# leonsick/depthg

Measured on AMD Instinct MI355X. Metric: correlation-loss steps/sec at B=32,C=384,28x28 (fwd+bwd, per-GPU batch 32), higher is better.
Workload: dtype bf16 (feats) / f16 (code) MFMA inputs, f32 accumulate

## Files before the change

depthg_amd/csrc/dg_corr_args.h:

```cpp
#pragma once
#include "dg_device.h"

__host__ __device__ inline int dg_perm32(int pl) {
    int s = pl >> 4, u = (pl >> 3) & 1, hh = (pl >> 2) & 1, v = pl & 3;
    return (2 * s + hh) * 8 + 4 * u + v;
}

#ifndef DG_F_IG
#define DG_F_IG 4
#endif
__host__ __device__ inline int dg_f_off(int q, int g) {
    constexpr int IG = DG_F_IG;
    return ((g / IG) * 32 + q) * (IG * 16) + (((g % IG) ^ ((q / (16 / IG)) % IG)) * 16);
}

struct DgBlob {
    int GF, GD, KD;
    int off_c, off_p, bytes;
    __host__ __device__ DgBlob(int KF, int KD_) : GF(KF / 8), GD(KD_ / 8), KD(KD_) {
        off_c = 32 * GF * 16;
        off_p = off_c + GD * 32 * 16;
        bytes = off_p + 4 * KD * 16;
    }
    __host__ __device__ int f(int q, int g) const { return dg_f_off(q, g); }
    __host__ __device__ int c(int q, int g) const { return off_c + (g * 32 + q) * 16; }
    __host__ __device__ int p(int d, int cc) const { return off_p + (cc * KD + d) * 16; }
};

template <int NKF, int NKD>
struct BlobT {
    static constexpr int KF = NKF * 16, KD = NKD * 16, GF = KF / 8, GD = KD / 8;
    static constexpr int OFF_C = 32 * GF * 16;
    static constexpr int OFF_P = OFF_C + GD * 32 * 16;
    static constexpr int BYTES = OFF_P + 4 * KD * 16;
    static constexpr int CHUNKS = BYTES / 1024;
    static constexpr int CHUNK_C0 = OFF_C / 1024;
    static constexpr int CHUNK_P0 = OFF_P / 1024;
    static_assert(BYTES % 1024 == 0 && OFF_C % 1024 == 0 && OFF_P % 1024 == 0, "blob parts must be KiB multiples");
    static_assert(GF % 16 == 0, "swizzle needs 16-granule groups");
};

__host__ __device__ inline size_t dg_gtile_off(int p, int d, int DP) {
    const int q = p & 31;
    return ((size_t)(p >> 5) * (DP >> 5) + (d >> 5)) * 1024 + (q >> 3) * 256 + ((d & 31) + 32 * ((q >> 2) & 1)) * 4 + (q & 3);
}

#define DG_XROWS_LDS (4 * 33 * 16)
template <int NDF>
__device__ __forceinline__ void dg_load_code_rows(const char* Cp, char* T, int lane, _Float16 (&x)[NDF][16]) {
        const int r = lane & 31, h = lane >> 5;
    i32x4 raw[NDF][2];
#pragma unroll
    for (int f = 0; f < NDF; ++f)
#pragma unroll
        for (int k = 0; k < 2; ++k) raw[f][k] = *reinterpret_cast<const i32x4*>(Cp + f * 2048 + k * 1024 + lane * 16);
#pragma unroll
    for (int f = 0; f < NDF; ++f) {
#pragma unroll
        for (int k = 0; k < 2; ++k) {
            const int L = k * 64 + lane;
            *reinterpret_cast<i32x4*>(T + ((L >> 5) * 33 + (L & 31)) * 16) = raw[f][k];
        }
#pragma unroll
        for (int i = 0; i < 16; ++i) {
            const int q = (i & 3) + 8 * (i >> 2) + 4 * h;
            x[f][i] = *reinterpret_cast<const _Float16*>(T + ((r >> 3) * 33 + q) * 16 + (r & 7) * 2);
        }
    }
}

enum { DG_JOB_HELPER = 0, DG_JOB_DEPTH = 1 };

struct DgJob {
    const char* Rop;
    const char* Sop;
    const float* rvec;
    const float* rimg;
    const uint32_t* maskbits;
    const float* nzR;
    const float* nzS;
    const float* RcInv;
    const float* Scsum;
    const int64_t* ridx;
    const int64_t* sidx;
    float* dR;
    float* part;
    float* out_cd;
    float* out_loss;
    uint16_t* Gout;
    float shift;
    int32_t kind;
    int32_t center_on_lane;
    int32_t slot_loss;
    int32_t slot_cd;
    float fin_scale;
    int32_t fold;
};

#define DG_MAX_JOBS 12
#define DG_GR_CAP 24

struct DgCorrArgs {
    DgJob jobs[DG_MAX_JOBS];
    int32_t njobs;
    int32_t B, P, Ppad;
    int32_t nrb;
    int32_t D;
    float lo, hi;
    float inv_BP;
    const char* dummy;
    int32_t pos_w;
    uint32_t* wctr;
    unsigned long long* span;
    int32_t half_tiles;
    uint32_t* stamps;
    unsigned long long* blocklog;
    const int32_t* gr_list;
    const int32_t* gr_count;
    const int16_t* gr_rank;
    int32_t gr_nkeys, gr_cpb;
    int32_t gr_blocks_per_image;
    int8_t gr_key[DG_MAX_JOBS];
    int8_t gr_first[DG_MAX_JOBS];
    int32_t gr_nblk[DG_MAX_JOBS];
};

struct DgFinishArgs {
    const float* part[DG_MAX_JOBS];
    int32_t slot_loss[DG_MAX_JOBS];
    int32_t slot_cd[DG_MAX_JOBS];
    float scale[DG_MAX_JOBS];
    int32_t njobs, nblk, B, P;
    int32_t nblk_job[DG_MAX_JOBS];
    const float* nzsum;
    float* out;
    float wtot[4];
};


struct DgTransposeArgs {
    const float* src[5];
    float* dst[5];
    int32_t K[5], K4[5], HW[5];
    int32_t nmaps;
};

struct DgGatherJob {
    const float* src;
    const float* coords;
    const int64_t* srcidx;
    char* blob;
    float* inv_norm;
    float* colpart;
    int32_t K, K4, Kpad;
    int32_t is_code;
    int32_t h, w;
    const float* ext_inv;
};
#define DG_MAX_GATHER 20
struct DgPreArgs {
    uint64_t seed; unsigned long long* state; int64_t* perms; int32_t count;
    const float* depth; float* nz; float* nzsum; int32_t dH, dW;
    const float* coords1; const float* coords2; char* taps;
    int32_t B, h, w, S, Sh, P, Ppad;
    unsigned int* zero_word;
};

struct DgCdMaskArgs {
    const float* rowsR;
    const float* rowsS[DG_MAX_NEG + 2];
    const int64_t* sidx[DG_MAX_NEG + 2];
    uint32_t* bits[DG_MAX_NEG + 2];
    int32_t T, B, P, Ppad, D, D4;
};

struct DgGatherArgs {
    DgGatherJob jobs[DG_MAX_GATHER];
    int32_t njobs, B, S, Sh, P, Ppad, KF, KD;
    int32_t direct;
    DgCdMaskArgs cd;
    int32_t cd_xper;
    DgPreArgs pre;
    int32_t pre_blocks, pre_nz, pre_z0;
};

struct DgPlaneArgs {
    const float* src[4];
    int32_t K[4], K4[4];
    float* rows[DG_MAX_NEG + 2][2];
    const float* coords1;
    const float* coords2;
    const int64_t* perms;
    int32_t nops, B, h, w, S, Sh, P;
    int32_t tap_consumers;
    int32_t feats_bf16;
    const float* src_x;
    float* rows_x;
};

__device__ __forceinline__ void dg_super_perm_row(const float* __restrict__ keys, uint64_t seed, unsigned long long* __restrict__ state,
                                                  int B, int64_t* __restrict__ out, int row, int nrows, float* sk) {
    const float* kr = keys ? keys + (size_t)row * B : nullptr;
    unsigned long long draw = 0;
    if (state) { seed = state[0]; draw = state[1]; }
    const uint64_t key = seed + 0x9E3779B97F4A7C15ull * draw;
    for (int i = threadIdx.x; i < B; i += 256)
        sk[i] = kr ? kr[i] : (float)(dg_philox(key, (uint32_t)(row * B + i)) >> 8) * (1.0f / 16777216.0f);
    __syncthreads();
    for (int i = threadIdx.x; i < B; i += 256) {
        const float ki = sk[i];
        int rank = 0;
        for (int j = 0; j < B; ++j) rank += (sk[j] < ki) || (sk[j] == ki && j < i);
        out[(size_t)row * B + rank] = (int64_t)((i == rank ? i + 1 : i) % B);
    }
    if (state && threadIdx.x == 0) {
        __threadfence();
        if (atomicAdd(&state[2], 1ull) == (unsigned long long)nrows - 1) {
            state[1] = draw + 1;
            state[2] = 0;
            __threadfence();
        }
    }
}

__device__ __forceinline__ float depth_nz_at(const float* __restrict__ depth, int n, int p, int H, int W, int Sh, int S) {
    float out = 0.f;
    if (p < Sh * S) {
        const int i = p / S, j = p - i * S;
        const float sy = Sh > 1 ? (float)(H - 1) / (float)(Sh - 1) : 0.f;
        const float sx = S > 1 ? (float)(W - 1) / (float)(S - 1) : 0.f;
        const float fy = dg_mul_rn(sy, (float)i), fx = dg_mul_rn(sx, (float)j);
        int y0 = min((int)fy, H - 1), x0 = min((int)fx, W - 1);
        const int y1 = y0 < H - 1 ? y0 + 1 : y0, x1 = x0 < W - 1 ? x0 + 1 : x0;
        const float ly1 = fy - (float)y0, lx1 = fx - (float)x0, ly0 = 1.f - ly1, lx0 = 1.f - lx1;
        const float* d = depth + (size_t)n * H * W;
        const float top = dg_mul_rn(d[(size_t)y0 * W + x0], lx0) + dg_mul_rn(d[(size_t)y0 * W + x1], lx1);
        const float bot = dg_mul_rn(d[(size_t)y1 * W + x0], lx0) + dg_mul_rn(d[(size_t)y1 * W + x1], lx1);
        const float v = dg_mul_rn(top, ly0) + dg_mul_rn(bot, ly1);
        out = v / fmaxf(fabsf(v), DG_EPS_NORM);
    }
    return out;
}

__device__ __forceinline__ void depth_nz_image(const float* __restrict__ depth, float* __restrict__ nz, float* __restrict__ nzsum,
                                               int n, int H, int W, int Sh, int S, int Ppad, bool pixel_order = false) {
    __shared__ float wred[4];
    float s = 0.f;
    for (int p = threadIdx.x; p < Ppad; p += 256) {
        const int pref = (pixel_order && p < Sh * S) ? (p % S) * S + p / S : p;
        const float v = depth_nz_at(depth, n, pref, H, W, Sh, S);
        nz[(size_t)n * Ppad + p] = v;
        s += v;
    }
#pragma unroll
    for (int o = 32; o > 0; o >>= 1) s += __shfl_xor(s, o, 64);
    if ((threadIdx.x & 63) == 0) wred[threadIdx.x >> 6] = s;
    __syncthreads();
    if (threadIdx.x == 0) nzsum[n] = wred[0] + wred[1] + wred[2] + wred[3];
}

struct DgSmallArgs {
    const void* rowsF[DG_MAX_NEG + 2];
    const float* rowsC[DG_MAX_NEG + 2];
    int32_t T, B, P, Ppad, C4, D, D4, KD;
    int32_t opR[DG_MAX_NEG + 2];
    int32_t opS[DG_MAX_NEG + 2];
    const int64_t* sidx[DG_MAX_NEG + 2];
    int32_t pointwise, depth, grad;
    float lo, hi;
    float shift[DG_MAX_NEG + 2], shift_depth;
    const float* nz;
    const float* nzsum;
    float* dRA[DG_MAX_NEG + 3];
    float* dRA2[DG_MAX_NEG + 2];
    float* dRB[DG_MAX_NEG + 2][2];
    float* dRB2[DG_MAX_NEG + 2][2];
    float* part;
    float* om;
    unsigned int* ticket;
    char* xop;
    float* xinv;
    int32_t blob_bytes, blob_off_c;
    float* out;
    float wtot[4];
    int32_t nsplit;
    float* out_cd;
    float* out_loss;
    int32_t mat_t, mat;
    int32_t debug;
    unsigned long long* span;
};

struct DgGatherRowsArgs {
    const float* src[2 * (DG_MAX_NEG + 2)];
    const float* coords[2 * (DG_MAX_NEG + 2)];
    const int64_t* srcidx[2 * (DG_MAX_NEG + 2)];
    void* rows[2 * (DG_MAX_NEG + 2)];
    int32_t K4[2 * (DG_MAX_NEG + 2)], h[2 * (DG_MAX_NEG + 2)], w[2 * (DG_MAX_NEG + 2)];
    int32_t Kout[2 * (DG_MAX_NEG + 2)], as_bf16[2 * (DG_MAX_NEG + 2)];
    int32_t njobs, B, S, Sh, P;
};

struct DgDenseArgs {
    const float* src[2];
    const float* code[2];
    char* blob[2];
    float* colpart[2];
    float* inv_norm[2];
    float* ccolpart[2];
    const float* depth;
    float* nz;
    float* nzsum;
    int32_t B, K, D, KF, KD, h, w, P, Ppad, dH, dW;
    int64_t* draw_out;
    unsigned long long* draw_state;
    uint64_t draw_seed;
    int32_t draw_count;
    int32_t code_split;
    const float* fkeep[2];
    float fscale;
    int32_t unit;
    int32_t roles;
};

struct DgDenseCodeArgs {
    const float* code[2];
    char* blob[2];
    const float* inv_norm[2];
    float* ccolpart[2];
    int32_t B, D, KF, KD, h, w, P, Ppad;
    char* clo[2];
};

struct DgGroupArgs {
    const int64_t* sidx[DG_MAX_JOBS];
    int8_t key[DG_MAX_JOBS];
    int32_t nh, nkeys, B;
    int32_t* list;
    int32_t* count;
    int16_t* rank;
};
__device__ __forceinline__ void dg_group_lists(const DgGroupArgs& g, const int m, const int key, const int lane) {
    const int B = g.B;
    int src[DG_MAX_JOBS];
#pragma unroll
    for (int j = 0; j < DG_MAX_JOBS; ++j) {
        const bool mine = j < g.nh && g.key[j] == key && lane < B;
        const int64_t* sidx = mine ? g.sidx[j] : nullptr;
        src[j] = mine ? (sidx ? (int)sidx[lane] : lane) : -1;
    }
    int cnt = 0;
#pragma unroll
    for (int j = 0; j < DG_MAX_JOBS; ++j) {
        const bool hit = src[j] == m;
        const unsigned long long mask = __ballot(hit);
        if (hit) {
            const int rk = cnt + __popcll(mask & ((1ull << lane) - 1ull));
            g.rank[j * B + lane] = (int16_t)(rk < 32767 ? rk : 32767);
            if (rk < DG_GR_CAP) g.list[(key * B + m) * DG_GR_CAP + rk] = j | (lane << 8);
        }
        cnt += __popcll(mask);
    }
    if (lane == 0) g.count[key * B + m] = cnt < DG_GR_CAP ? cnt : DG_GR_CAP;
}

struct DgColmeanArgs {
    const float* colpart[DG_MAX_NEG + 2];
    float* bbar[DG_MAX_NEG + 2];
    __bf16* bsplit[DG_MAX_NEG + 2];
    const float* ccolpart[DG_MAX_NEG + 2];
    float* csum[DG_MAX_NEG + 2];
// ... 154 lines not shown
```

depthg_amd/csrc/dg_post.hip:

```cpp
#include "dg_device.h"
#include "dg_corr_args.h"
#include "dg_taps.h"
#include <cstdlib>

typedef const float __attribute__((address_space(1)))* gfloat_p;


#define DG_LOAD_GS(a, gs)                                                                                   \
    float gs[4];                                                                                            \
    {                                                                                                       \
        const bool vec_ = (a).gscal != nullptr;                                                             \
        const float gt_ = vec_ ? (a).gscal[DG_OUT_TOTAL] : (a).gtot[0];                                     \
        const float g0_ = vec_ ? (a).gscal[0] : 0.f, g1_ = vec_ ? (a).gscal[1] : 0.f;                       \
        const float g2_ = vec_ ? (a).gscal[2] : 0.f, g3_ = vec_ ? (a).gscal[3] : 0.f;                       \
        gs[0] = g0_ + gt_ * (a).wtot[0]; gs[1] = g1_ + gt_ * (a).wtot[1];                                  \
        gs[2] = g2_ + gt_ * (a).wtot[2]; gs[3] = g3_ + gt_ * (a).wtot[3];                                  \
    }
__device__ __forceinline__ float dg_pick(const float (&gs)[4], int i) { return i == 0 ? gs[0] : (i == 1 ? gs[1] : (i == 2 ? gs[2] : gs[3])); }

template <int NDF>
__global__ __launch_bounds__(64 * NDF) void k_grad_combine(const DgScatterArgs a) {
    const int rt = blockIdx.x, n = blockIdx.y, dest = blockIdx.z;
    const int lane = threadIdx.x & 63, r = lane & 31, h = lane >> 5, DP = NDF * 32;
    const int d = __builtin_amdgcn_readfirstlane((int)threadIdx.x >> 6);
    if (dest >= 2) {
        const int j = dest - 2;
        const size_t off = ((size_t)n * (a.Ppad >> 5) + rt) * (32 * DP) + d * 1024 + lane * 4;
        const float f = a.axf[j] ? a.axf[j][0] : 0.f;
        const float* const d2 = a.axd2[j];
        const float* const s1 = a.axs[j];
        const float* const s2 = a.axs2[j];
        f32x4 y[4], y2[4], x[4], x2[4];
#pragma unroll
        for (int g = 0; g < 4; ++g) {
            y[g] = *reinterpret_cast<const f32x4*>(a.axd[j] + off + g * 256);
            y2[g] = d2 ? *reinterpret_cast<const f32x4*>(d2 + off + g * 256) : f32x4{0.f, 0.f, 0.f, 0.f};
            x[g] = s1 ? *reinterpret_cast<const f32x4*>(s1 + off + g * 256) : f32x4{0.f, 0.f, 0.f, 0.f};
            x2[g] = s2 ? *reinterpret_cast<const f32x4*>(s2 + off + g * 256) : f32x4{0.f, 0.f, 0.f, 0.f};
        }
#pragma unroll
        for (int g = 0; g < 4; ++g) {
#pragma unroll
            for (int e = 0; e < 4; ++e) y[g][e] = fmaf(f, x[g][e] + x2[g][e], y[g][e] + y2[g][e]);
            *reinterpret_cast<f32x4*>(a.axo[j] + off + g * 256) = y[g];
        }
        return;
    }
    __shared__ __attribute__((aligned(16))) char xs[NDF][DG_XROWS_LDS];
    __shared__ float part[NDF][32];
    DG_LOAD_GS(a, gs)
    const bool ok = 32 * d + r < a.D;
    const size_t tile_off = ((size_t)n * (a.Ppad >> 5) + rt) * (32 * DP) + lane * 4 + (ok ? d * 1024 : 0);
    float v[16];
#pragma unroll
    for (int i = 0; i < 16; ++i) v[i] = 0.f;
    auto add_sources = [&](const int8_t* list, const int cnt) __attribute__((always_inline)) {
        for (int k0 = 0; k0 < cnt; k0 += 4) {
            f32x4 t[4][4];
            float sc[4];
#pragma unroll
            for (int u = 0; u < 4; ++u) {
                const bool live = k0 + u < cnt;
                const DgScatterSrc& q = a.src[(int)list[live ? k0 + u : k0]];
                sc[u] = live ? dg_src_factor(q) * dg_pick(gs, q.gidx) : 0.f;
                const float* base = q.buf + tile_off;
#pragma unroll
                for (int g = 0; g < 4; ++g) t[u][g] = *reinterpret_cast<const f32x4*>(base + (ok ? g * 256 : 0));
            }
#pragma unroll
            for (int u = 0; u < 4; ++u) {
                const bool use = ok && k0 + u < cnt;
#pragma unroll
                for (int g = 0; g < 4; ++g)
#pragma unroll
                    for (int e = 0; e < 4; ++e) v[4 * g + e] = fmaf(sc[u], use ? t[u][g][e] : 0.f, v[4 * g + e]);
            }
        }
    };
    const int nraw = a.ncraw[dest];
    add_sources(a.craw[dest], nraw);
    if (nraw > 0) {
        const char* xb = a.xop + ((size_t)n * (a.Ppad >> 5) + rt) * a.blob_bytes + a.blob_off_c + d * 2048;
        _Float16 x[1][16];
        dg_load_code_rows<1>(xb, xs[d], lane, x);
#pragma unroll
        for (int i = 0; i < 16; ++i) {
            const float t = half_sum((float)x[0][i] * v[i]);
            if (r == 0) part[d][h * 16 + i] = t;
        }
        __syncthreads();
#pragma unroll
        for (int i = 0; i < 16; ++i) {
            float t = part[0][h * 16 + i];
#pragma unroll
            for (int f = 1; f < NDF; ++f) t += part[f][h * 16 + i];
            const int rr = rt * 32 + (i & 3) + 8 * (i >> 2) + 4 * h;
            const float inv = rr < a.P ? a.xinv[(size_t)n * a.Ppad + rr] : 0.f;
            v[i] = (v[i] - (float)x[0][i] * t) * inv;
        }
    }
    add_sources(a.cfin[dest], a.ncfin[dest]);
    if (ok) {
        float* out = a.comb[dest] + tile_off;
#pragma unroll
        for (int g = 0; g < 4; ++g) {
            const f32x4 t = {v[4 * g], v[4 * g + 1], v[4 * g + 2], v[4 * g + 3]};
            *reinterpret_cast<f32x4*>(out + g * 256) = t;
        }
    }
}

#ifndef COMB_HB_HM
#define COMB_HB_HM 4
#endif
#ifndef COMB_HB
#define COMB_HB 4
#endif
#define COMB_MAXROUTE 512
template <int NDF, bool HM = false>
__global__ __launch_bounds__(64 * NDF) void k_combine_out(const DgScatterArgs a) {
    const int rt = blockIdx.x, n = blockIdx.y, dest = blockIdx.z;
    const int tid = threadIdx.x, lane = tid & 63, r = lane & 31, h = lane >> 5, DP = NDF * 32;
    const int d = __builtin_amdgcn_readfirstlane(tid >> 6);
    __shared__ __attribute__((aligned(16))) char xs[NDF][DG_XROWS_LDS];
    __shared__ float part[NDF][32];
    __shared__ float stage[NDF][32 * 33];
    __shared__ const float* rl_p[COMB_MAXROUTE];
    __shared__ float rl_w[COMB_MAXROUTE];
    __shared__ int rl_cnt, wcnt[NDF], rsrc[DG_MAX_SCATTER];
    DG_LOAD_GS(a, gs)
    int nr = 0;
    for (int s = 0; s < a.nsrc; ++s)
        if (a.src[s].dest == dest && a.src[s].route != nullptr) { if (tid == 0) rsrc[nr] = s; ++nr; }
    if (tid == 0) rl_cnt = 0;
    __syncthreads();
    for (int i0 = 0; i0 < nr * a.B; i0 += 64 * NDF) {
        const int i = i0 + tid;
        bool hit = false;
        int m = 0, s = 0;
        if (i < nr * a.B) {
            const int rs = i / a.B;
            m = i - rs * a.B; s = rsrc[rs];
            hit = (int)a.src[s].route[m] == n;
        }
        const unsigned long long bal = __ballot(hit);
        if (lane == 0) wcnt[d] = __popcll(bal);
        __syncthreads();
        int base = rl_cnt;
        for (int wv = 0; wv < d; ++wv) base += wcnt[wv];
        if (hit) {
            const int o = base + __popcll(bal & ((1ull << lane) - 1));
            const DgScatterSrc& q = a.src[s];
            if (o < COMB_MAXROUTE) {
                rl_p[o] = q.half ? reinterpret_cast<const float*>(reinterpret_cast<const _Float16*>(q.buf) + (size_t)m * a.Ppad * a.DP) : q.buf + (size_t)m * a.Ppad * a.DP;
                rl_w[o] = dg_src_factor(q) * dg_pick(gs, q.gidx);
            }
        }
        __syncthreads();
        if (tid == 0) {
            int c = rl_cnt;
            for (int wv = 0; wv < NDF; ++wv) c += wcnt[wv];
            rl_cnt = min(c, COMB_MAXROUTE);
        }
        __syncthreads();
    }
    const int cnt = rl_cnt;
    const bool ok = 32 * d + r < a.D;
    const size_t in_img = (size_t)rt * (32 * DP) + lane * 4 + (ok ? d * 1024 : 0);
    const size_t tile_off = (size_t)n * a.Ppad * DP + in_img;
    float v[16];
#pragma unroll
    for (int i = 0; i < 16; ++i) v[i] = 0.f;
    const size_t in_img_h = (size_t)rt * (32 * DP) + lane * 8 + (ok ? d * 1024 : 0);
    constexpr int HB = HM ? COMB_HB_HM : COMB_HB, FB = HM ? 1 : 4;
    float invd[16];
#pragma unroll
    for (int i = 0; i < 16; ++i) {
        const int rr = rt * 32 + (i & 3) + 8 * (i >> 2) + 4 * h;
        invd[i] = (a.xinv_dest[dest] && rr < a.P) ? a.xinv_dest[dest][(size_t)n * a.Ppad + rr] : 0.f;
    }
    const _Float16 __attribute__((address_space(1)))* const hdummy = reinterpret_cast<const _Float16 __attribute__((address_space(1)))*>(reinterpret_cast<uintptr_t>(a.xinv));
    auto add_half4 = [&](const _Float16 __attribute__((address_space(1)))* const (&hb)[HB], const float (&sc)[HB], const bool raw) __attribute__((always_inline)) {
        f16x8 t0[HB], t1[HB];
#pragma unroll
        for (int u = 0; u < HB; ++u) {
            t0[u] = *reinterpret_cast<const f16x8 __attribute__((address_space(1)))*>(hb[u]);
            t1[u] = *reinterpret_cast<const f16x8 __attribute__((address_space(1)))*>(hb[u] + ((ok && hb[u] != hdummy) ? 512 : 0));
        }
#pragma unroll
        for (int u = 0; u < HB; ++u) {
            const bool use = ok && sc[u] != 0.f;
#pragma unroll
            for (int e = 0; e < 8; ++e) {
                v[e] = fmaf(raw ? sc[u] : sc[u] * invd[e], use ? (float)t0[u][e] : 0.f, v[e]);
                v[8 + e] = fmaf(raw ? sc[u] : sc[u] * invd[8 + e], use ? (float)t1[u][e] : 0.f, v[8 + e]);
            }
        }
    };
    auto add_sources_half = [&](const int8_t* list, const int nsrc_, const bool raw) __attribute__((always_inline)) {
        for (int k0 = 0; k0 < nsrc_; k0 += HB) {
            const _Float16 __attribute__((address_space(1)))* hb[HB];
            float sc[HB];
#pragma unroll
            for (int u = 0; u < HB; ++u) {
                const bool live = k0 + u < nsrc_;
                const DgScatterSrc& q = a.src[(int)list[live ? k0 + u : k0]];
                sc[u] = live ? dg_src_factor(q) * dg_pick(gs, q.gidx) : 0.f;
                hb[u] = live ? reinterpret_cast<const _Float16 __attribute__((address_space(1)))*>(reinterpret_cast<uintptr_t>(q.buf)) + (size_t)n * a.Ppad * DP + in_img_h
                             : hdummy;
            }
            add_half4(hb, sc, raw);
        }
    };
    auto add_sources = [&](const int8_t* list, const int nsrc_) __attribute__((always_inline)) {

        for (int k0 = 0; k0 < nsrc_; k0 += FB) {
            f32x4 t[FB][4];
            float sc[FB];
#pragma unroll
            for (int u = 0; u < FB; ++u) {
                const bool live = k0 + u < nsrc_;
                const DgScatterSrc& q = a.src[(int)list[live ? k0 + u : k0]];
                sc[u] = live ? dg_src_factor(q) * dg_pick(gs, q.gidx) : 0.f;
                const float* base = q.buf + tile_off;
#pragma unroll
                for (int g = 0; g < 4; ++g) t[u][g] = *reinterpret_cast<const f32x4*>(base + (ok ? g * 256 : 0));
            }
#pragma unroll
            for (int u = 0; u < FB; ++u) {
                const bool use = ok && k0 + u < nsrc_;
#pragma unroll
                for (int g = 0; g < 4; ++g)
#pragma unroll
                    for (int e = 0; e < 4; ++e) v[4 * g + e] = fmaf(sc[u], use ? t[u][g][e] : 0.f, v[4 * g + e]);
            }
        }
    };
    const int nraw = a.ncraw[dest] + a.ncrawh[dest];
    add_sources(a.craw[dest], a.ncraw[dest]);
    add_sources_half(a.crawh[dest], a.ncrawh[dest], true);
    if (nraw > 0) {
        const char* xb = a.xop + ((size_t)n * (a.Ppad >> 5) + rt) * a.blob_bytes + a.blob_off_c + d * 2048;
        _Float16 x[1][16];
        dg_load_code_rows<1>(xb, xs[d], lane, x);
#pragma unroll
        for (int i = 0; i < 16; ++i) {
            const float t = half_sum((float)x[0][i] * v[i]);
            if (r == 0) part[d][h * 16 + i] = t;
        }
        __syncthreads();
#pragma unroll
        for (int i = 0; i < 16; ++i) {
            float t = part[0][h * 16 + i];
#pragma unroll
            for (int f = 1; f < NDF; ++f) t += part[f][h * 16 + i];
            const int rr = rt * 32 + (i & 3) + 8 * (i >> 2) + 4 * h;
            const float inv = rr < a.P ? a.xinv[(size_t)n * a.Ppad + rr] : 0.f;
            v[i] = (v[i] - (float)x[0][i] * t) * inv;
        }
    }
    add_sources(a.cfin[dest], a.ncfin[dest]);
    add_sources_half(a.cfinh[dest], a.ncfinh[dest], false);
    if (a.routed_half) {
        for (int e0 = 0; e0 < cnt; e0 += HB) {
            const _Float16 __attribute__((address_space(1)))* hb[HB];
            float sc[HB];
#pragma unroll
            for (int k = 0; k < HB; ++k) {
                const int e = min(e0 + k, cnt - 1);
                sc[k] = e0 + k < cnt ? rl_w[e] : 0.f;
                hb[k] = sc[k] != 0.f ? reinterpret_cast<const _Float16 __attribute__((address_space(1)))*>(reinterpret_cast<uintptr_t>(rl_p[e])) + in_img_h : hdummy;
            }
            add_half4(hb, sc, false);
        }
    } else
    for (int e0 = 0; e0 < cnt; e0 += 4) {
        f32x4 u4[4][4];
        float sc[4];
#pragma unroll
        for (int k = 0; k < 4; ++k) {
            const int e = min(e0 + k, cnt - 1);
            sc[k] = e0 + k < cnt ? rl_w[e] : 0.f;
            const gfloat_p sb = (gfloat_p)rl_p[e] + in_img;
#pragma unroll
            for (int g = 0; g < 4; ++g) u4[k][g] = *(const f32x4 __attribute__((address_space(1)))*)(sb + (ok ? g * 256 : 0));
        }
#pragma unroll
        for (int k = 0; k < 4; ++k)
#pragma unroll
            for (int g = 0; g < 4; ++g)
#pragma unroll
                for (int e = 0; e < 4; ++e) v[4 * g + e] = fmaf(sc[k], ok ? u4[k][g][e] : 0.f, v[4 * g + e]);
    }
    float* st = stage[d];
#pragma unroll
    for (int i = 0; i < 16; ++i) st[r * 33 + (i & 3) + 8 * (i >> 2) + 4 * h] = v[i];
    __builtin_amdgcn_fence(__ATOMIC_RELEASE, "workgroup");
    __builtin_amdgcn_wave_barrier();
    __builtin_amdgcn_fence(__ATOMIC_ACQUIRE, "workgroup");
    const int HW = a.h * a.w, p = rt * 32 + r;
    float* out = a.out[dest] + (size_t)n * a.D * HW + p;
#pragma unroll
    for (int it = 0; it < 16; ++it) {
        const int c = 2 * it + h, ch = 32 * d + c;
        if (ch < a.D && p < a.P) out[(size_t)ch * HW] = st[c * 33 + r];
    }
}

#define SCAT_THREADS 1024
#define SCAT_DC 4
#define SCAT_PX (SCAT_THREADS / SCAT_DC)
#define SCAT_MAXPASS 16

__global__ __launch_bounds__(SCAT_THREADS) void k_build_taps(const DgScatterArgs a) {
    extern __shared__ __attribute__((aligned(16))) char sg[];
    const DgTapsArgs t{a.coords1, a.coords2, a.taps, a.B, a.h, a.w, a.S, a.Sh, a.P};
    build_taps_block<SCAT_THREADS>(t, (int)blockIdx.x, (int)blockIdx.y, sg);
}

__global__ __launch_bounds__(256) void k_pre_general(const DgPreArgs a) {
    extern __shared__ __attribute__((aligned(16))) char pg[];
    int b = (int)blockIdx.x;
    if (a.zero_word && b == 0 && threadIdx.x == 0) *a.zero_word = 0u;
    if (b < a.count) { dg_super_perm_row(nullptr, a.seed, a.state, a.B, a.perms, b, a.count, reinterpret_cast<float*>(pg)); return; }
    b -= a.count;
    if (a.depth) {
        if (b < a.B) { depth_nz_image(a.depth, a.nz, a.nzsum, b, a.dH, a.dW, a.Sh, a.S, a.Ppad); return; }
        b -= a.B;
    }
    if (!a.taps) return;
    const DgTapsArgs t{a.coords1, a.coords2, a.taps, a.B, a.h, a.w, a.S, a.Sh, a.P};
    build_taps_block<256>(t, b % a.B, b / a.B, pg);
}

hipError_t dg_launch_pre_general(const DgPreArgs& a, hipStream_t s) {
    int nblk = a.count + (a.depth ? a.B : 0) + (a.taps ? 2 * a.B : 0);
    if (nblk == 0 && a.zero_word) nblk = 1;
    if (nblk == 0) return hipSuccess;
    size_t smem = a.count > 0 ? (size_t)a.B * 4 : 0;
    if (a.taps) {
        const size_t need = dg_taps_record_bytes(a.h * a.w, a.P) + (size_t)a.h * a.w * 4 + 16;
        smem = need > smem ? need : smem;
    }
    return dg_launch(k_pre_general, dim3(nblk), dim3(256), (int)smem, s, a);
}

#define SCAT_RMAX 8
template <int NPASS>
__global__ __launch_bounds__(SCAT_THREADS) void k_scatter_grad(const DgScatterArgs a, int rmax) {
    extern __shared__ __attribute__((aligned(16))) char sg[];
    const int tid = threadIdx.x, HW = a.h * a.w, P = a.P;
    const int aD = a.D, aDP = a.DP, aB = a.B, aPpad = a.Ppad;
    const char* const taps_base = a.taps;
    DG_LOAD_GS(a, gs)
    const int dc0 = blockIdx.x * SCAT_DC, bdst = blockIdx.y, dest = blockIdx.z;
    const int dl = tid & (SCAT_DC - 1), px = tid / SCAT_DC, d = dc0 + dl;
    const int npass = (HW + SCAT_PX - 1) / SCAT_PX;
    const size_t rec = dg_taps_record_bytes(HW, P);
    __shared__ const float* b_src[SCAT_RMAX];
    __shared__ const char* b_rec[SCAT_RMAX];
    __shared__ float b_sc[SCAT_RMAX];
    float acc[NPASS];
#pragma unroll
    for (int i = 0; i < NPASS; ++i) acc[i] = 0.f;
    int npend = 0;

    auto flush = [&, aD, aDP]() __attribute__((always_inline)) {
        if (npend == 0) return;
        __syncthreads();
        const int n16 = (int)(rec / 16);
        for (int i = tid; i < npend * n16; i += SCAT_THREADS) {
            const int r = i / n16, k = i - r * n16;
            reinterpret_cast<f32x4*>(sg)[i] = *((const f32x4 __attribute__((address_space(1)))*)b_rec[r] + k);
        }
        __syncthreads();
        if (d < aD) {
            const int DPc = aDP;
            constexpr int RG = NPASS <= 4 ? 4 : (NPASS <= 8 ? 2 : 1);
            for (int r0 = 0; r0 < npend; r0 += RG) {
                float v[RG][NPASS], w[RG][NPASS];
                int e0[RG][NPASS];
#pragma unroll
                for (int g = 0; g < RG; ++g) {
                    const int r = min(r0 + g, npend - 1);
                    const int* off = reinterpret_cast<const int*>(sg + (size_t)r * rec);
                    const float* ewgt = reinterpret_cast<const float*>(off + HW + 1);
                    const unsigned short* eidx = reinterpret_cast<const unsigned short*>(ewgt + 4 * P);
                    const gfloat_p src = (gfloat_p)b_src[r];
#pragma unroll
                    for (int ps = 0; ps < NPASS; ++ps) {
                        const int pix = ps * SCAT_PX + px;
                        const bool ok = r0 + g < npend && ps < npass && pix < HW;
                        const int ea = ok ? off[pix] : 0, eb = ok ? off[pix + 1] : 0;
                        const bool any = eb > ea;
                        w[g][ps] = any ? ewgt[ea] : 0.f;
                        v[g][ps] = any ? src[dg_gtile_off(eidx[ea], d, DPc)] : 0.f;
                        e0[g][ps] = ea | (eb > ea + 1 ? (int)0x80000000 : 0);
                    }
                }
#pragma unroll
                for (int g = 0; g < RG; ++g) {
                    if (r0 + g < npend) {
                        const int r = r0 + g;
                        const int* off = reinterpret_cast<const int*>(sg + (size_t)r * rec);
                        const float* ewgt = reinterpret_cast<const float*>(off + HW + 1);
                        const unsigned short* eidx = reinterpret_cast<const unsigned short*>(ewgt + 4 * P);
                        const gfloat_p src = (gfloat_p)b_src[r];
                        const float sc = b_sc[r];
#pragma unroll
                        for (int ps = 0; ps < NPASS; ++ps) {
                            float sum = w[g][ps] * v[g][ps];
                            if (e0[g][ps] < 0) {
                                const int ea = e0[g][ps] & 0x7fffffff, eb = off[ps * SCAT_PX + px + 1];
                                for (int e = ea + 1; e < eb; ++e) sum = fmaf(ewgt[e], src[dg_gtile_off(eidx[e], d, DPc)], sum);
                            }
                            acc[ps] = fmaf(sc, sum, acc[ps]);
                        }
                    }
                }
            }
        }
        __syncthreads();
        npend = 0;
    };
    auto push = [&](const float* buf, float sc, int cs, int nimg) __attribute__((always_inline)) {
        if (tid == 0) {
            b_src[npend] = buf + (size_t)nimg * aPpad * aDP;
            b_rec[npend] = taps_base + ((size_t)cs * aB + nimg) * rec;
            b_sc[npend] = sc;
        }
        if (++npend == rmax) flush();
    };

    push(a.comb[dest], 1.0f, dest == 0 ? 0 : 1, bdst);
    for (int s = 0; s < a.nsrc; ++s) {
        const DgScatterSrc& q = a.src[s];
        if (q.dest != dest || q.route == nullptr) continue;
        const float sc = dg_src_factor(q) * dg_pick(gs, q.gidx);
        for (int n0 = 0; n0 < a.B; n0 += 64) {
            const int nn = n0 + (tid & 63);
            const bool hit = nn < a.B && (int)q.route[nn] == bdst;
            unsigned long long m = __ballot(hit);
            while (m) {
                const int n = n0 + __builtin_ctzll(m);
                m &= m - 1;
                push(q.buf, sc, q.coords_sel, n);
            }
        }
    }
    flush();
    float* stage = reinterpret_cast<float*>(sg);
#pragma unroll
    for (int ps = 0; ps < NPASS; ++ps) {
        const int pix = ps * SCAT_PX + px;
        if (ps < npass && pix < HW) stage[dl * (HW + 1) + pix] = acc[ps];
    }
    __syncthreads();
    float* out = a.out[dest];
    for (int i = tid; i < SCAT_DC * HW; i += SCAT_THREADS) {
        const int dd = i / HW, pix = i - dd * HW;
        if (dc0 + dd < a.D) out[((size_t)bdst * a.D + dc0 + dd) * HW + pix] = stage[dd * (HW + 1) + pix];
    }
}

template <int CG>
__global__ __launch_bounds__(SCAT_THREADS) void k_scatter_small(const DgScatterArgs a, int rb) {
    constexpr int VS = CG + 1;
    extern __shared__ __attribute__((aligned(16))) char sg[];
    const int tid = threadIdx.x, HW = a.h * a.w, P = a.P, nt = a.Ppad >> 5, NF = a.DP >> 5;
    const int aB = a.B, aPpad = a.Ppad, aDP = a.DP;
    const char* const taps_base = a.taps;
    DG_LOAD_GS(a, gs)
    const int f = blockIdx.x / (32 / CG), cg = blockIdx.x % (32 / CG), bdst = blockIdx.y, dest = blockIdx.z;
    const size_t rec = dg_taps_record_bytes(HW, P);
    const int vstride = aPpad * VS;
    float* const vals = reinterpret_cast<float*>(sg + (size_t)rb * rec);
    __shared__ const float* b_src[SCAT_RMAX];
    __shared__ const char* b_rec[SCAT_RMAX];
    __shared__ float b_sc[SCAT_RMAX];
    float acc[CG];
#pragma unroll
    for (int c = 0; c < CG; ++c) acc[c] = 0.f;
    int npend = 0;

    auto flush = [&, rec, nt, NF, f, cg, vstride, HW, P]() __attribute__((always_inline)) {
        if (npend == 0) return;
        __syncthreads();
        const int n16 = (int)(rec / 16);
        for (int i = tid; i < npend * n16; i += SCAT_THREADS) {
            const int r = i / n16, k = i - r * n16;
            reinterpret_cast<f32x4*>(sg)[i] = *((const f32x4 __attribute__((address_space(1)))*)b_rec[r] + k);
        }
        constexpr int PT = 8 * CG;
        for (int i = tid; i < npend * nt * PT; i += SCAT_THREADS) {
            const int r = i / (nt * PT), j = i - r * (nt * PT), t = j / PT, k = j - t * PT;
            const int c = k % CG, hq = k / CG;
            const int jj = (hq >> 1) * 64 + (hq & 1) * 32 + CG * cg + c;
            const f32x4 v = *((const f32x4 __attribute__((address_space(1)))*)(b_src[r] + ((size_t)t * NF + f) * 1024) + jj);
            float* o = vals + (size_t)r * vstride + (t * 32 + hq * 4) * VS + c;
            o[0] = v[0]; o[VS] = v[1]; o[2 * VS] = v[2]; o[3 * VS] = v[3];
        }
        __syncthreads();
        if (tid < HW) {
            for (int r = 0; r < npend; ++r) {
                const int* off = reinterpret_cast<const int*>(sg + (size_t)r * rec);
                const float* ewgt = reinterpret_cast<const float*>(off + HW + 1);
                const unsigned short* eidx = reinterpret_cast<const unsigned short*>(ewgt + 4 * P);
                const float* vr = vals + (size_t)r * vstride;
                const int e0 = off[tid], e1 = off[tid + 1];
                const float sc = b_sc[r];
                for (int e = e0; e < e1; ++e) {
                    const float w = sc * ewgt[e];
                    const float* v = vr + (int)eidx[e] * VS;
#pragma unroll
                    for (int c = 0; c < CG; ++c) acc[c] = fmaf(w, v[c], acc[c]);
                }
            }
        }
        __syncthreads();
        npend = 0;
    };
    auto push = [&](const float* buf, float sc, int cs, int nimg) __attribute__((always_inline)) {
        if (tid == 0) {
            b_src[npend] = buf + (size_t)nimg * aPpad * aDP;
            b_rec[npend] = taps_base + ((size_t)cs * aB + nimg) * rec;
            b_sc[npend] = sc;
        }
        if (++npend == rb) flush();
    };
    __shared__ short l_s[16 * 64 + 1], l_n[16 * 64 + 1];
    for (int n0 = 0; n0 < a.B; n0 += 64) {
        const int nn = n0 + (tid & 63);
        for (int s0 = 0; s0 < a.nsrc || s0 == 0; s0 += 16) {
            int cnt = 0;
            if (n0 == 0 && s0 == 0) { if (tid == 0) { l_s[0] = -1; l_n[0] = (short)bdst; } cnt = 1; }
            int rt[16];
#pragma unroll
            for (int k = 0; k < 16; ++k) {
                const int s = s0 + k;
                const bool use = s < a.nsrc && a.src[s < a.nsrc ? s : 0].dest == dest && a.src[s < a.nsrc ? s : 0].route != nullptr && nn < a.B;
                rt[k] = use ? (int)a.src[s].route[nn] : -1;
            }
#pragma unroll
            for (int k = 0; k < 16; ++k) {
                const unsigned long long m = __ballot(rt[k] == bdst);
                if (tid == 0) {
                    int c = cnt;
                    for (unsigned long long mm = m; mm; mm &= mm - 1) { l_s[c] = (short)(s0 + k); l_n[c] = (short)(n0 + __builtin_ctzll(mm)); ++c; }
                }
                cnt += __popcll(m);
            }
            __syncthreads();
            for (int i = 0; i < cnt; ++i) {
                const int s = l_s[i], n = l_n[i];
                const DgScatterSrc& q = a.src[s < 0 ? 0 : s];
                const float* buf = s < 0 ? a.comb[dest] : q.buf;
                const float sc = s < 0 ? 1.0f : dg_src_factor(q) * dg_pick(gs, q.gidx);
                const int cs = s < 0 ? (dest == 0 ? 0 : 1) : q.coords_sel;
                push(buf, sc, cs, n);
            }
            __syncthreads();
        }
    }
    flush();
    if (tid < HW) {
        const int d0 = 32 * f + CG * cg;
        float* out = a.out[dest] + ((size_t)bdst * a.D + d0) * HW + tid;
#pragma unroll
        for (int c = 0; c < CG; ++c)
            if (d0 + c < a.D) out[(size_t)c * HW] = acc[c];
    }
}

#define DENSE_MAXROUTE 1024
template <int CG, int DENSE_THREADS>
__global__ __launch_bounds__(DENSE_THREADS) void k_scatter_dense(const DgScatterArgs a) {
    extern __shared__ __attribute__((aligned(16))) char sd[];
    const int HW = a.h * a.w, nt = a.Ppad >> 5, NF = a.DP >> 5;
    DG_LOAD_GS(a, gs)
    float* stage = reinterpret_cast<float*>(sd);
    const float** rl_p = reinterpret_cast<const float**>(stage + CG * (HW + 2));
    float* rl_w = reinterpret_cast<float*>(rl_p + DENSE_MAXROUTE);
    __shared__ int rl_cnt;
    constexpr int TPW = 32 / CG;
    const int f = blockIdx.x / TPW, cg = blockIdx.x % TPW, b = blockIdx.y, dest = blockIdx.z;
    const int tid = threadIdx.x, lane = tid & 63, wid = tid >> 6;
    const int ts = lane / (2 * CG), h = (lane / CG) & 1, idx = lane % CG;
    const int r = CG * cg + idx;
    constexpr int NW = DENSE_THREADS / 64;
    __shared__ int wcnt[NW];
    __shared__ int rsrc[DG_MAX_SCATTER];
    int nr = 0;
    for (int s = 0; s < a.nsrc; ++s)
        if (a.src[s].dest == dest && a.src[s].route != nullptr) { if (tid == 0) rsrc[nr] = s; ++nr; }
    if (tid == 0) rl_cnt = 0;
// ... 434 lines not shown
```

Measured before the change: 3374.

## Overlap route scan with raw-source and code-row loads in combine_out

Restructures k_combine_out so each wave builds its routed-source list on its own, using ballots and wave-local counts instead of block-wide syncthreads rounds. The first batch of raw-source loads and the code-row loads are issued before the route scan so their latency overlaps with it. Per-row inverse norms are now loaded once per lane and spread with shuffles instead of 16 scattered global loads. It adds register pressure from the shared staging buffer, and the routed list is now built per wave, which duplicates the route scan across waves.

```diff
diff --git a/depthg_amd/csrc/dg_corr_args.h b/depthg_amd/csrc/dg_corr_args.h
--- a/depthg_amd/csrc/dg_corr_args.h
+++ b/depthg_amd/csrc/dg_corr_args.h
@@ -47,13 +47,15 @@
 
 #define DG_XROWS_LDS (4 * 33 * 16)
 template <int NDF>
-__device__ __forceinline__ void dg_load_code_rows(const char* Cp, char* T, int lane, _Float16 (&x)[NDF][16]) {
-        const int r = lane & 31, h = lane >> 5;
-    i32x4 raw[NDF][2];
+__device__ __forceinline__ void dg_request_code_rows(const char* Cp, int lane, i32x4 (&raw)[NDF][2]) {
 #pragma unroll
     for (int f = 0; f < NDF; ++f)
 #pragma unroll
         for (int k = 0; k < 2; ++k) raw[f][k] = *reinterpret_cast<const i32x4*>(Cp + f * 2048 + k * 1024 + lane * 16);
+}
+template <int NDF>
+__device__ __forceinline__ void dg_turn_code_rows(const i32x4 (&raw)[NDF][2], char* T, int lane, _Float16 (&x)[NDF][16]) {
+    const int r = lane & 31, h = lane >> 5;
 #pragma unroll
     for (int f = 0; f < NDF; ++f) {
 #pragma unroll
@@ -67,6 +69,12 @@
             x[f][i] = *reinterpret_cast<const _Float16*>(T + ((r >> 3) * 33 + q) * 16 + (r & 7) * 2);
         }
     }
+}
+template <int NDF>
+__device__ __forceinline__ void dg_load_code_rows(const char* Cp, char* T, int lane, _Float16 (&x)[NDF][16]) {
+    i32x4 raw[NDF][2];
+    dg_request_code_rows<NDF>(Cp, lane, raw);
+    dg_turn_code_rows<NDF>(raw, T, lane, x);
 }
 
 enum { DG_JOB_HELPER = 0, DG_JOB_DEPTH = 1 };
diff --git a/depthg_amd/csrc/dg_post.hip b/depthg_amd/csrc/dg_post.hip
--- a/depthg_amd/csrc/dg_post.hip
+++ b/depthg_amd/csrc/dg_post.hip
@@ -117,6 +117,7 @@
 #define COMB_HB 4
 #endif
 #define COMB_MAXROUTE 512
+#define COMB_BALLOTS 4
 template <int NDF, bool HM = false>
 __global__ __launch_bounds__(64 * NDF) void k_combine_out(const DgScatterArgs a) {
     const int rt = blockIdx.x, n = blockIdx.y, dest = blockIdx.z;
@@ -127,44 +128,37 @@
     __shared__ float stage[NDF][32 * 33];
     __shared__ const float* rl_p[COMB_MAXROUTE];
     __shared__ float rl_w[COMB_MAXROUTE];
-    __shared__ int rl_cnt, wcnt[NDF], rsrc[DG_MAX_SCATTER];
+    __shared__ const int64_t* rs_route[DG_MAX_SCATTER];
+    __shared__ const float* rs_buf[DG_MAX_SCATTER];
+    __shared__ float rs_w[DG_MAX_SCATTER];
     DG_LOAD_GS(a, gs)
     int nr = 0;
-    for (int s = 0; s < a.nsrc; ++s)
-        if (a.src[s].dest == dest && a.src[s].route != nullptr) { if (tid == 0) rsrc[nr] = s; ++nr; }
-    if (tid == 0) rl_cnt = 0;
-    __syncthreads();
-    for (int i0 = 0; i0 < nr * a.B; i0 += 64 * NDF) {
-        const int i = i0 + tid;
-        bool hit = false;
-        int m = 0, s = 0;
-        if (i < nr * a.B) {
-            const int rs = i / a.B;
-            m = i - rs * a.B; s = rsrc[rs];
-            hit = (int)a.src[s].route[m] == n;
-        }
-        const unsigned long long bal = __ballot(hit);
-        if (lane == 0) wcnt[d] = __popcll(bal);
-        __syncthreads();
-        int base = rl_cnt;
-        for (int wv = 0; wv < d; ++wv) base += wcnt[wv];
-        if (hit) {
-            const int o = base + __popcll(bal & ((1ull << lane) - 1));
-            const DgScatterSrc& q = a.src[s];
-            if (o < COMB_MAXROUTE) {
-                rl_p[o] = q.half ? reinterpret_cast<const float*>(reinterpret_cast<const _Float16*>(q.buf) + (size_t)m * a.Ppad * a.DP) : q.buf + (size_t)m * a.Ppad * a.DP;
-                rl_w[o] = dg_src_factor(q) * dg_pick(gs, q.gidx);
-            }
-        }
-        __syncthreads();
-        if (tid == 0) {
-            int c = rl_cnt;
-            for (int wv = 0; wv < NDF; ++wv) c += wcnt[wv];
-            rl_cnt = min(c, COMB_MAXROUTE);
-        }
-        __syncthreads();
-    }
-    const int cnt = rl_cnt;
+    for (int s = 0; s < a.nsrc; ++s) {
+        const DgScatterSrc& q = a.src[s];
+        if (q.dest == dest && q.route != nullptr) {
+            if (lane == 0) { rs_route[nr] = q.route; rs_buf[nr] = q.buf; rs_w[nr] = dg_src_factor(q) * dg_pick(gs, q.gidx); }
+            ++nr;
+        }
+    }
+    __builtin_amdgcn_fence(__ATOMIC_RELEASE, "workgroup");
+    __builtin_amdgcn_wave_barrier();
+    __builtin_amdgcn_fence(__ATOMIC_ACQUIRE, "workgroup");
+    const int npairs = min(nr * a.B, COMB_MAXROUTE);
+    int rdst[COMB_BALLOTS];
+    auto request_routes = [&](const int i0) __attribute__((always_inline)) {
+#pragma unroll
+        for (int k = 0; k < COMB_BALLOTS; ++k) {
+            rdst[k] = -1;
+            if (i0 + 64 * k < npairs) {
+                const unsigned i = i0 + 64 * k + lane;
+                if (i < (unsigned)npairs) {
+                    const unsigned rs = i / (unsigned)a.B;
+                    rdst[k] = (int)((const int64_t __attribute__((address_space(1)))*)rs_route[rs])[i - rs * a.B];
+                }
+            }
+        }
+    };
+    request_routes(0);
     const bool ok = 32 * d + r < a.D;
     const size_t in_img = (size_t)rt * (32 * DP) + lane * 4 + (ok ? d * 1024 : 0);
     const size_t tile_off = (size_t)n * a.Ppad * DP + in_img;
@@ -173,76 +167,110 @@
     for (int i = 0; i < 16; ++i) v[i] = 0.f;
     const size_t in_img_h = (size_t)rt * (32 * DP) + lane * 8 + (ok ? d * 1024 : 0);
     constexpr int HB = HM ? COMB_HB_HM : COMB_HB, FB = HM ? 1 : 4;
+    const float invd_r = (a.xinv_dest[dest] && rt * 32 + r < a.P) ? a.xinv_dest[dest][(size_t)n * a.Ppad + rt * 32 + r] : 0.f;
     float invd[16];
-#pragma unroll
-    for (int i = 0; i < 16; ++i) {
-        const int rr = rt * 32 + (i & 3) + 8 * (i >> 2) + 4 * h;
-        invd[i] = (a.xinv_dest[dest] && rr < a.P) ? a.xinv_dest[dest][(size_t)n * a.Ppad + rr] : 0.f;
-    }
     const _Float16 __attribute__((address_space(1)))* const hdummy = reinterpret_cast<const _Float16 __attribute__((address_space(1)))*>(reinterpret_cast<uintptr_t>(a.xinv));
-    auto add_half4 = [&](const _Float16 __attribute__((address_space(1)))* const (&hb)[HB], const float (&sc)[HB], const bool raw) __attribute__((always_inline)) {
-        f16x8 t0[HB], t1[HB];
+    constexpr int TB = 4 * FB > 2 * HB ? 4 * FB : 2 * HB;
+    i32x4 tb[TB];
+    float sch[HB];
+    auto request_half = [&](const _Float16 __attribute__((address_space(1)))* const (&hb)[HB]) __attribute__((always_inline)) {
 #pragma unroll
         for (int u = 0; u < HB; ++u) {
-            t0[u] = *reinterpret_cast<const f16x8 __attribute__((address_space(1)))*>(hb[u]);
-            t1[u] = *reinterpret_cast<const f16x8 __attribute__((address_space(1)))*>(hb[u] + ((ok && hb[u] != hdummy) ? 512 : 0));
-        }
+            tb[2 * u] = *reinterpret_cast<const i32x4 __attribute__((address_space(1)))*>(hb[u]);
+            tb[2 * u + 1] = *reinterpret_cast<const i32x4 __attribute__((address_space(1)))*>(hb[u] + ((ok && hb[u] != hdummy) ? 512 : 0));
+        }
+    };
+    auto sum_half = [&](const bool raw) __attribute__((always_inline)) {
 #pragma unroll
         for (int u = 0; u < HB; ++u) {
-            const bool use = ok && sc[u] != 0.f;
+            const bool use = ok && sch[u] != 0.f;
+            const f16x8 t0 = __builtin_bit_cast(f16x8, tb[2 * u]), t1 = __builtin_bit_cast(f16x8, tb[2 * u + 1]);
 #pragma unroll
             for (int e = 0; e < 8; ++e) {
-                v[e] = fmaf(raw ? sc[u] : sc[u] * invd[e], use ? (float)t0[u][e] : 0.f, v[e]);
-                v[8 + e] = fmaf(raw ? sc[u] : sc[u] * invd[8 + e], use ? (float)t1[u][e] : 0.f, v[8 + e]);
-            }
-        }
-    };
-    auto add_sources_half = [&](const int8_t* list, const int nsrc_, const bool raw) __attribute__((always_inline)) {
-        for (int k0 = 0; k0 < nsrc_; k0 += HB) {
-            const _Float16 __attribute__((address_space(1)))* hb[HB];
-            float sc[HB];
-#pragma unroll
-            for (int u = 0; u < HB; ++u) {
-                const bool live = k0 + u < nsrc_;
-                const DgScatterSrc& q = a.src[(int)list[live ? k0 + u : k0]];
-                sc[u] = live ? dg_src_factor(q) * dg_pick(gs, q.gidx) : 0.f;
-                hb[u] = live ? reinterpret_cast<const _Float16 __attribute__((address_space(1)))*>(reinterpret_cast<uintptr_t>(q.buf)) + (size_t)n * a.Ppad * DP + in_img_h
-                             : hdummy;
-            }
-            add_half4(hb, sc, raw);
-        }
-    };
-    auto add_sources = [&](const int8_t* list, const int nsrc_) __attribute__((always_inline)) {
-
-        for (int k0 = 0; k0 < nsrc_; k0 += FB) {
-            f32x4 t[FB][4];
-            float sc[FB];
-#pragma unroll
-            for (int u = 0; u < FB; ++u) {
-                const bool live = k0 + u < nsrc_;
-                const DgScatterSrc& q = a.src[(int)list[live ? k0 + u : k0]];
-                sc[u] = live ? dg_src_factor(q) * dg_pick(gs, q.gidx) : 0.f;
-                const float* base = q.buf + tile_off;
-#pragma unroll
-                for (int g = 0; g < 4; ++g) t[u][g] = *reinterpret_cast<const f32x4*>(base + (ok ? g * 256 : 0));
-            }
-#pragma unroll
-            for (int u = 0; u < FB; ++u) {
-                const bool use = ok && k0 + u < nsrc_;
-#pragma unroll
-                for (int g = 0; g < 4; ++g)
-#pragma unroll
-                    for (int e = 0; e < 4; ++e) v[4 * g + e] = fmaf(sc[u], use ? t[u][g][e] : 0.f, v[4 * g + e]);
-            }
-        }
-    };
-    const int nraw = a.ncraw[dest] + a.ncrawh[dest];
-    add_sources(a.craw[dest], a.ncraw[dest]);
-    add_sources_half(a.crawh[dest], a.ncrawh[dest], true);
+                v[e] = fmaf(raw ? sch[u] : sch[u] * invd[e], use ? (float)t0[e] : 0.f, v[e]);
+                v[8 + e] = fmaf(raw ? sch[u] : sch[u] * invd[8 + e], use ? (float)t1[e] : 0.f, v[8 + e]);
+            }
+        }
+    };
+    auto request_sources_half = [&](const int8_t* list, const int k0, const int nsrc_) __attribute__((always_inline)) {
+        const _Float16 __attribute__((address_space(1)))* hb[HB];
+#pragma unroll
+        for (int u = 0; u < HB; ++u) {
+            const bool live = k0 + u < nsrc_;
+            const DgScatterSrc& q = a.src[(int)list[live ? k0 + u : k0]];
+            sch[u] = live ? dg_src_factor(q) * dg_pick(gs, q.gidx) : 0.f;
+            hb[u] = live ? reinterpret_cast<const _Float16 __attribute__((address_space(1)))*>(reinterpret_cast<uintptr_t>(q.buf)) + (size_t)n * a.Ppad * DP + in_img_h
+                         : hdummy;
+        }
+        request_half(hb);
+    };
+    float scf[FB];
+    auto request_sources = [&](const int8_t* list, const int k0, const int nsrc_) __attribute__((always_inline)) {
+#pragma unroll
+        for (int u = 0; u < FB; ++u) {
+            const bool live = k0 + u < nsrc_;
+            const DgScatterSrc& q = a.src[(int)list[live ? k0 + u : k0]];
+            scf[u] = live ? dg_src_factor(q) * dg_pick(gs, q.gidx) : 0.f;
+            const float* base = q.buf + tile_off;
+#pragma unroll
+            for (int g = 0; g < 4; ++g) tb[4 * u + g] = *reinterpret_cast<const i32x4*>(base + (ok ? g * 256 : 0));
+        }
+    };
+    auto sum_sources = [&](const int k0, const int nsrc_) __attribute__((always_inline)) {
+#pragma unroll
+        for (int u = 0; u < FB; ++u) {
+            const bool use = ok && k0 + u < nsrc_;
+#pragma unroll
+            for (int g = 0; g < 4; ++g) {
+                const f32x4 t = __builtin_bit_cast(f32x4, tb[4 * u + g]);
+#pragma unroll
+                for (int e = 0; e < 4; ++e) v[4 * g + e] = fmaf(scf[u], use ? t[e] : 0.f, v[4 * g + e]);
+            }
+        }
+    };
+    const int nrawf = a.ncraw[dest], nrawh = a.ncrawh[dest], nraw = nrawf + nrawh;
+    float xinv_r = 0.f;
+    i32x4 xraw[1][2];
     if (nraw > 0) {
-        const char* xb = a.xop + ((size_t)n * (a.Ppad >> 5) + rt) * a.blob_bytes + a.blob_off_c + d * 2048;
+        if (rt * 32 + r < a.P) xinv_r = a.xinv[(size_t)n * a.Ppad + rt * 32 + r];
+        dg_request_code_rows<1>(a.xop + ((size_t)n * (a.Ppad >> 5) + rt) * a.blob_bytes + a.blob_off_c + d * 2048, lane, xraw);
+    }
+    if (nrawf > 0) request_sources(a.craw[dest], 0, nrawf);
+    else if (nrawh > 0) request_sources_half(a.crawh[dest], 0, nrawh);
+    int cnt = 0;
+    for (int i0 = 0; i0 < npairs; i0 += 64 * COMB_BALLOTS) {
+        if (i0 > 0) request_routes(i0);
+#pragma unroll
+        for (int k = 0; k < COMB_BALLOTS; ++k) {
+            if (i0 + 64 * k < npairs) {
+                const bool hit = rdst[k] == n;
+                const unsigned long long bal = __ballot(hit);
+                const int o = cnt + __popcll(bal & ((1ull << lane) - 1));
+                if (hit && o < COMB_MAXROUTE) {
+                    const unsigned i = i0 + 64 * k + lane, rs = i / (unsigned)a.B;
+                    const size_t img = (size_t)(i - rs * a.B) * a.Ppad * a.DP;
+                    rl_p[o] = a.routed_half ? reinterpret_cast<const float*>(reinterpret_cast<const _Float16*>(rs_buf[rs]) + img) : rs_buf[rs] + img;
+                    rl_w[o] = rs_w[rs];
+                }
+                cnt += __popcll(bal);
+            }
+        }
+    }
+    cnt = min(cnt, COMB_MAXROUTE);
+    __builtin_amdgcn_fence(__ATOMIC_RELEASE, "workgroup");
+    __builtin_amdgcn_wave_barrier();
+    __builtin_amdgcn_fence(__ATOMIC_ACQUIRE, "workgroup");
+    for (int k0 = 0; k0 < nrawf; k0 += FB) {
+        if (k0 > 0) request_sources(a.craw[dest], k0, nrawf);
+        sum_sources(k0, nrawf);
+    }
+    for (int k0 = 0; k0 < nrawh; k0 += HB) {
+        if (k0 > 0 || nrawf > 0) request_sources_half(a.crawh[dest], k0, nrawh);
+        sum_half(true);
+    }
+    if (nraw > 0) {
         _Float16 x[1][16];
-        dg_load_code_rows<1>(xb, xs[d], lane, x);
+        dg_turn_code_rows<1>(xraw, xs[d], lane, x);
 #pragma unroll
         for (int i = 0; i < 16; ++i) {
             const float t = half_sum((float)x[0][i] * v[i]);
@@ -254,43 +282,53 @@
             float t = part[0][h * 16 + i];
 #pragma unroll
             for (int f = 1; f < NDF; ++f) t += part[f][h * 16 + i];
-            const int rr = rt * 32 + (i & 3) + 8 * (i >> 2) + 4 * h;
-            const float inv = rr < a.P ? a.xinv[(size_t)n * a.Ppad + rr] : 0.f;
+            const float inv = __shfl(xinv_r, (i & 3) + 8 * (i >> 2) + 4 * h);
             v[i] = (v[i] - (float)x[0][i] * t) * inv;
         }
     }
-    add_sources(a.cfin[dest], a.ncfin[dest]);
-    add_sources_half(a.cfinh[dest], a.ncfinh[dest], false);
+#pragma unroll
+    for (int i = 0; i < 16; ++i) invd[i] = __shfl(invd_r, (i & 3) + 8 * (i >> 2) + 4 * h);
+    for (int k0 = 0; k0 < a.ncfin[dest]; k0 += FB) {
+        request_sources(a.cfin[dest], k0, a.ncfin[dest]);
+        sum_sources(k0, a.ncfin[dest]);
+    }
+    for (int k0 = 0; k0 < a.ncfinh[dest]; k0 += HB) {
+        request_sources_half(a.cfinh[dest], k0, a.ncfinh[dest]);
+        sum_half(false);
+    }
     if (a.routed_half) {
         for (int e0 = 0; e0 < cnt; e0 += HB) {
             const _Float16 __attribute__((address_space(1)))* hb[HB];
-            float sc[HB];
 #pragma unroll
             for (int k = 0; k < HB; ++k) {
                 const int e = min(e0 + k, cnt - 1);
+                sch[k] = e0 + k < cnt ? rl_w[e] : 0.f;
+                hb[k] = sch[k] != 0.f ? reinterpret_cast<const _Float16 __attribute__((address_space(1)))*>(reinterpret_cast<uintptr_t>(rl_p[e])) + in_img_h : hdummy;
+            }
+            request_half(hb);
+            sum_half(false);
+        }
+    } else {
+        constexpr int RB = TB / 4;
+        for (int e0 = 0; e0 < ((cnt + 3) & ~3); e0 += RB) {
+            float sc[RB];
+#pragma unroll
+            for (int k = 0; k < RB; ++k) {
+                const int e = min(e0 + k, cnt - 1);
                 sc[k] = e0 + k < cnt ? rl_w[e] : 0.f;
-                hb[k] = sc[k] != 0.f ? reinterpret_cast<const _Float16 __attribute__((address_space(1)))*>(reinterpret_cast<uintptr_t>(rl_p[e])) + in_img_h : hdummy;
-            }
-            add_half4(hb, sc, false);
-        }
-    } else
-    for (int e0 = 0; e0 < cnt; e0 += 4) {
-        f32x4 u4[4][4];
-        float sc[4];
-#pragma unroll
-        for (int k = 0; k < 4; ++k) {
-            const int e = min(e0 + k, cnt - 1);
-            sc[k] = e0 + k < cnt ? rl_w[e] : 0.f;
-            const gfloat_p sb = (gfloat_p)rl_p[e] + in_img;
-#pragma unroll
-            for (int g = 0; g < 4; ++g) u4[k][g] = *(const f32x4 __attribute__((address_space(1)))*)(sb + (ok ? g * 256 : 0));
-        }
-#pragma unroll
-        for (int k = 0; k < 4; ++k)
-#pragma unroll
-            for (int g = 0; g < 4; ++g)
-#pragma unroll
-                for (int e = 0; e < 4; ++e) v[4 * g + e] = fmaf(sc[k], ok ? u4[k][g][e] : 0.f, v[4 * g + e]);
+                const gfloat_p sb = (gfloat_p)rl_p[e] + in_img;
+#pragma unroll
+                for (int g = 0; g < 4; ++g) tb[4 * k + g] = *(const i32x4 __attribute__((address_space(1)))*)(sb + (ok ? g * 256 : 0));
+            }
+#pragma unroll
+            for (int k = 0; k < RB; ++k)
+#pragma unroll
+                for (int g = 0; g < 4; ++g) {
+                    const f32x4 t = __builtin_bit_cast(f32x4, tb[4 * k + g]);
+#pragma unroll
+                    for (int e = 0; e < 4; ++e) v[4 * g + e] = fmaf(sc[k], ok ? t[e] : 0.f, v[4 * g + e]);
+                }
+        }
     }
     float* st = stage[d];
 #pragma unroll
```

Measured after the change: 3427 (median of 6 runs). +1.6%, better.
